# a-slide/Quade

Measured on AMD Instinct MI355X. Metric: read-pairs/sec demultiplexed (2x150 bp, dual 8 bp index), higher is better.
Workload: dtype u8

## Files before the change

quade_amd/csrc/quade_inflate3.hip:

```cpp
#include <hip/hip_runtime.h>
#include <stdint.h>
#include <stdio.h>
#include <stdlib.h>

#include "crc_lds.h"
#include "quade_inflate.h"
#include "inflate3_lane.h"
#include "quade_inflate3.h"
#include "quade_pool.h"

namespace {

using CfgS = qd3::Cfg<7, 6, 88, true, 8, 12>;
using CfgA = qd3::Cfg<8, 7, 112>;
static_assert((CfgS::LANE_DW * 64 + CfgS::RING_DW) * 4 * 4 <= 160 * 1024 - 2048, "four workgroups per CU");
static_assert((CfgA::LANE_DW * 64 + CfgA::RING_DW) * 4 * 2 <= 160 * 1024, "two workgroups per CU");

template <class C, int WPB>
__global__ __launch_bounds__(64 * WPB) void inflate3_tokens(const qd3::Unit* units, const qd_inflate3_job* jobs, uint32_t n_units, uint16_t* tokens, uint32_t* lens_scratch,
                                                            qd3::Result* res, uint32_t wait_rounds, uint32_t redo) {
    extern __shared__ __attribute__((aligned(16))) uint32_t lds_all[];
    const uint32_t lane = threadIdx.x & 63u, wave = (uint32_t)__builtin_amdgcn_readfirstlane((int)(threadIdx.x >> 6));
    uint32_t* const lds3 = lds_all + wave * (uint32_t)(C::LANE_DW * 64 + C::RING_DW);
    uint32_t* const ring = lds3;
    uint16_t* const tab = reinterpret_cast<uint16_t*>(lds3 + C::RING_DW + lane * (uint32_t)C::LANE_DW);
#pragma unroll 1
  for (uint32_t group = blockIdx.x * (uint32_t)WPB + wave; 64u * group < n_units; group += gridDim.x * (uint32_t)WPB) {
    const uint32_t u = 64u * group + lane;
    bool mine = u < n_units;
    if (redo) {
        mine = mine && res[u].status == (uint32_t)QD_INFLATE_TABLE_SPACE;
        if (!__ballot(mine)) continue;
    }
    qd3::Lane<C> L;
    {
        qd3::Unit un{nullptr, 0, ~0ull, 0, 0, 0, 0, nullptr, 0, 0};
        if (mine) {
            if (jobs) {
                const qd_inflate3_job j = jobs[u];
                const uintptr_t a = reinterpret_cast<uintptr_t>(j.payload);
                un.base = reinterpret_cast<const uint32_t*>(a & ~(uintptr_t)15);
                un.bit_start = 8ull * (a & 15u);
                un.bit_end = un.bit_start + 8ull * j.in_len;
                un.tok_off = (uint64_t)u * QD_INFLATE3_TOK_STRIDE;
                un.tok_cap = QD_INFLATE3_TOK_STRIDE;
                un.wend = (uint32_t)(((a & 15u) + j.in_len + 3u) / 4u) + 80u;
            } else {
                un = units[u];
            }
        }
        qd3::lane_init(L, un, lens_scratch + (size_t)(mine ? u : 0) * qd3::LENS_DW);
        if (!mine) {
            L.state = qd3::ST_DONE;
            L.status = 0;
        }
    }
    qd3::topup(L, ring, lane, mine);
    qd3::ring_wait();
    qd3::landed_all(L);
    qd3::prime(L, ring, lane);
    uint32_t waited = 0;
#pragma unroll 1
    for (;;) {
        const bool hdr = L.state == qd3::ST_HEADER, dec = L.state <= qd3::ST_STORED;
        const uint64_t mh = __ballot(hdr), md = __ballot(dec);
        if (!mh && !md) break;
        if (mh && (!md || waited >= wait_rounds)) {
            qd3::topup(L, ring, lane, hdr);
            qd3::ring_wait();
            qd3::landed_all(L);
            if (hdr) qd3::header<C>(L, tab, ring, lane);
            qd3::topup(L, ring, lane, L.state <= qd3::ST_STORED);
            qd3::ring_wait();
            qd3::landed_all(L);
            waited = 0;
            continue;
        }
        if (dec && qd3::bitpos(L) > L.bit_end + 64u) qd3::fail(L, QD_INFLATE_TRUNCATED);
        qd3::ring_wait();
        qd3::landed_all(L);
        qd3::topup(L, ring, lane, dec);
        if (__ballot(L.state == qd3::ST_STORED)) {
#pragma unroll 1
            for (int t = 0; t < C::ROUND_TURNS; ++t) {
                if (L.state == qd3::ST_STORED) qd3::turn_stored<C>(L, ring, lane, tokens);
                else if (L.state <= qd3::ST_DIST) qd3::turn<C>(L, tab, ring, lane, tokens);
            }
        } else {
#pragma unroll 1
            for (int t = 0; t < C::ROUND_TURNS; ++t)
                if (L.state <= qd3::ST_DIST) qd3::turn<C>(L, tab, ring, lane, tokens);
        }
        if (mh) ++waited;
    }
    if (mine) qd3::lane_finish(L, res + u);
  }
}

template <int NT, int Q>
struct R3Lds {
    uint32_t ow[16384 + 4];
    uint16_t par[Q];
    uint32_t wsum[NT / 64 + 1];
    uint32_t ctl[8];
};

template <int NT>
__device__ __forceinline__ uint32_t block_scan_excl(uint32_t v, uint32_t* wsum, uint32_t& total) {
    const uint32_t lane = threadIdx.x & 63u, wave = threadIdx.x >> 6;
    uint32_t inc = v;
#pragma unroll
    for (int d = 1; d < 64; d <<= 1) {
        const uint32_t y = __shfl_up(inc, d, 64);
        if (lane >= (uint32_t)d) inc += y;
    }
    if (lane == 63) wsum[wave] = inc;
    __syncthreads();
    uint32_t base = 0, tot = 0;
#pragma unroll
    for (int w = 0; w < NT / 64; ++w) {
        const uint32_t s = wsum[w];
        if ((uint32_t)w < wave) base += s;
        tot += s;
    }
    __syncthreads();
    total = tot;
    return base + inc - v;
}

template <int NT, int Q>
__global__ __launch_bounds__(NT) void inflate3_resolve_bgzf(const qd_inflate3_job* jobs, uint32_t n_blocks, const uint16_t* tokens, const qd3::Result* res,
                                                            int32_t* status) {
    static_assert(Q % NT == 0 && Q / NT <= 32 && 65536 % Q == 0, "a lane's share of a window");
    static_assert((size_t)Q * 2 >= 4096 + (NT / 64) * 4, "the CRC stage's tables lie where the parents were");
    constexpr int K = Q / NT;
    constexpr int CRC_SW = NT >= 1024 ? 17 : (NT >= 512 ? 33 : 65);
    static_assert((size_t)NT * CRC_SW * 4 >= 65536, "the CRC stage's slices");
    extern __shared__ __attribute__((aligned(16))) uint8_t lds_raw3[];
    R3Lds<NT, Q>& S = *reinterpret_cast<R3Lds<NT, Q>*>(lds_raw3);
    uint8_t* const ob = reinterpret_cast<uint8_t*>(S.ow);
    typedef volatile __attribute__((address_space(3))) uint8_t lds_vu8;
    typedef volatile __attribute__((address_space(3))) uint16_t lds_vu16;
    lds_vu8* const vob = (lds_vu8*)ob;
    lds_vu16* const par = (lds_vu16*)S.par;
    const uint32_t i = blockIdx.x, tid = threadIdx.x;
    if (i >= n_blocks) return;
    const qd_inflate3_job blk = jobs[i];
    const qd3::Result r = res[i];
    const uint32_t olen = blk.out_len;
    int err = (int)r.status;
    if (!err && olen > 65536u) err = QD_INFLATE_OVERRUN;
    if (!err && !r.final_seen) err = QD_INFLATE_BAD_TYPE;
    if (!err && r.text_len != olen) err = r.text_len > olen ? QD_INFLATE_OVERRUN : QD_INFLATE_LENGTH;
    if (!err && r.bit_next > 8ull * ((reinterpret_cast<uintptr_t>(blk.payload) & 15u) + (uint64_t)blk.in_len)) err = QD_INFLATE_TRUNCATED;
    if (tid < 8) S.ctl[tid] = 0;
    __syncthreads();
    if (!err) {
        const uint16_t* tk = tokens + (size_t)i * QD_INFLATE3_TOK_STRIDE;
        const uint32_t n_slots = r.n_slots;
        auto init_par = [&](uint32_t w) {
            const uint32_t qb = w * Q;
#pragma unroll
            for (int k = 0; k < K; ++k) {
                const uint32_t p = qb + tid + (uint32_t)k * NT;
                par[p - qb] = (uint16_t)p;
            }
            __syncthreads();
        };
        auto finalize = [&](uint32_t w) {
            const uint32_t qb = w * Q, hi = min(qb + (uint32_t)Q, olen);
            if (tid == 0) S.ctl[5] = S.ctl[6] = S.ctl[7] = 0;
            __syncthreads();
            uint32_t pend = 0;
#pragma unroll
            for (int k = 0; k < K; ++k) {
                const uint32_t p = qb + tid + (uint32_t)k * NT;
                if (p < hi && par[p - qb] != (uint16_t)p) pend |= 1u << k;
            }
            constexpr int MATCH_ROUNDS = 24;
#pragma unroll 1
            for (int round = 0; round < MATCH_ROUNDS; ++round) {
#pragma unroll 1
                for (uint32_t left = pend; left; left &= left - 1u) {
                    const uint32_t k = (uint32_t)__builtin_ctz(left), p = qb + tid + k * NT;
                    const uint32_t q = par[p - qb];
                    if (q < qb || par[q - qb] == q) {
                        vob[p] = vob[q];
                        par[p - qb] = (uint16_t)p;
                        pend &= ~(1u << k);
                    } else {
                        par[p - qb] = par[q - qb];
                    }
                }
                uint32_t* flag = &S.ctl[5];
                if (pend) flag[round % 3] = 1;
                __syncthreads();
                const uint32_t more = flag[round % 3];
                if (tid == 0) flag[(round + 2) % 3] = 0;
                if (!more) break;
                if (round == MATCH_ROUNDS - 1 && tid == 0) S.ctl[4] = 1;
            }
            __syncthreads();
        };
        uint32_t base_pos = 0, cur_win = 0;
        init_par(0);
#pragma unroll 1
        for (uint32_t c0 = 0; c0 < n_slots; c0 += NT * 4u) {
            const uint32_t s0 = c0 + 4u * tid;
            uint64_t four = 0;
            uint32_t prev = 0, next = 0;
            if (s0 < n_slots) {
                four = *reinterpret_cast<const uint64_t*>(tk + s0);
                if (s0) prev = tk[s0 - 1];
                if (s0 + 4u < n_slots) next = tk[s0 + 4u];
            }
            uint32_t sl[5], ln[4], at[4], sum = 0;
#pragma unroll
            for (int j = 0; j < 4; ++j) sl[j] = (uint32_t)(four >> (16 * j)) & 0xFFFFu;
            sl[4] = next;
#pragma unroll
            for (int j = 0; j < 4; ++j) {
                const bool valid = s0 + (uint32_t)j < n_slots;
                const bool is_dist = ((j ? sl[j - 1] : prev) & qd3::TOK_MATCH) != 0;
                ln[j] = (!valid || is_dist) ? 0u : ((sl[j] & qd3::TOK_MATCH) ? (sl[j] & 0xFFu) + 3u : 1u);
                sum += ln[j];
            }
            uint32_t total;
            uint32_t pos = base_pos + block_scan_excl<NT>(sum, S.wsum, total);
#pragma unroll
            for (int j = 0; j < 4; ++j) {
                at[j] = pos;
                if (ln[j] == 1u && pos < olen) ob[pos] = (uint8_t)sl[j];
                pos += ln[j];
            }
            const uint32_t chunk_hi = min(base_pos + total, olen);
            const uint32_t w_first = cur_win, w_last = max(w_first, chunk_hi ? (chunk_hi - 1u) / (uint32_t)Q : 0u);
#pragma unroll 1
            for (uint32_t w = w_first; w <= w_last; ++w) {
                if (w != cur_win) {
                    finalize(cur_win);
                    cur_win = w;
                    init_par(w);
                }
                const uint32_t wlo = w * Q, whi = min(wlo + (uint32_t)Q, olen);
#pragma unroll
                for (int j = 0; j < 4; ++j) {
                    if (ln[j] < 3u) continue;
                    const uint32_t d0 = at[j], len = ln[j], dist = sl[j + 1] + 1u;
                    if (dist > d0 || d0 + len > olen) {
                        S.ctl[4] = 1;
                        continue;
                    }
                    const uint32_t a = max(d0, wlo), z = min(d0 + len, whi);
                    for (uint32_t p = a; p < z; ++p) par[p - wlo] = (uint16_t)(p - dist);
                }
            }
            base_pos += total;
        }
        finalize(cur_win);
        if (S.ctl[4]) err = QD_INFLATE_BAD_DISTANCE;
    }
    __syncthreads();
    if (blk.check_crc) {
        uint32_t* crc_t = reinterpret_cast<uint32_t*>(S.par);
        qdcrc::stage_tables<NT>(crc_t);
        __syncthreads();
        const uint32_t crc = qdcrc::crc32_lds<NT, CRC_SW>(S.ow, err ? 0u : olen, crc_t, crc_t + 1024);
        if (!err && crc != blk.expect_crc) err = QD_INFLATE_CRC;
    }
    if (!err) {
        uint8_t* const o = blk.out;
        const uint32_t head = min(olen, (uint32_t)((4u - ((uintptr_t)o & 3u)) & 3u));
        if (tid < head) o[tid] = ob[tid];
        const uint32_t nd = (olen - head) >> 2;
        for (uint32_t k = tid; k < nd; k += NT) {
            const uint32_t a = head + 4 * k, wi = a >> 2;
            *reinterpret_cast<uint32_t*>(o + a) = __builtin_amdgcn_alignbyte(S.ow[wi + 1], S.ow[wi], a & 3u);
        }
        for (uint32_t k = head + 4 * nd + tid; k < olen; k += NT) o[k] = ob[k];
    }
    if (tid == 0) status[i] = err;
}

struct GzStretch {
    const uint32_t* base;
    uint64_t bit_from;
    uint64_t bit_to;
    uint64_t bit_end;
};

__device__ __forceinline__ uint64_t gz_bits(const uint32_t* base, uint64_t bit) {
    const uint64_t w = bit >> 5;
    const uint32_t sh = (uint32_t)bit & 31u;
    const uint64_t lo = base[w], mid = base[w + 1], hi = base[w + 2];
    return sh ? ((lo | (mid << 32)) >> sh) | (hi << (64u - sh)) : (lo | (mid << 32));
}

__device__ __forceinline__ bool gz_text_lengths_only(uint32_t a, uint32_t b) {
    b = min(b, 256u);
    if (a >= b) return true;
    const uint64_t non_text[4] = {0x00000000FFFFD9FFull, 0x8000000000000000ull, ~0ull, ~0ull};
    bool hit = false;
#pragma unroll
    for (uint32_t w = 0; w < 4; ++w) {
        const uint32_t lo = max(a, 64u * w), hi = min(b, 64u * w + 64u);
        if (lo < hi) {
            const uint64_t bits = (hi - lo == 64u ? ~0ull : ((1ull << (hi - lo)) - 1ull)) << (lo - 64u * w);
            hit = hit || (non_text[w] & bits) != 0;
        }
    }
    return !hit;
}
__device__ bool gz_header_holds(const uint32_t* base, uint64_t bit, uint64_t bit_end, uint8_t* clt, bool text_only) {
    if (bit + 17 + 12 > bit_end) return false;
    uint64_t x = gz_bits(base, bit);
    if ((x & 7u) != 4u) return false;
    const uint32_t nlit = ((uint32_t)(x >> 3) & 31u) + 257u, ndist = ((uint32_t)(x >> 8) & 31u) + 1u, ncl = ((uint32_t)(x >> 13) & 15u) + 4u;
    if (nlit > 286u || ndist > 30u) return false;
    uint64_t pos = bit + 17;
    x = gz_bits(base, pos);
    uint64_t cl = 0, cc = 0;
    for (uint32_t k = 0; k < ncl; ++k) {
        const uint32_t sym = (uint32_t)((k < 12 ? qd3::CLORDER_LO >> (5u * k) : qd3::CLORDER_HI >> (5u * (k - 12u))) & 31u);
        const uint32_t l = (uint32_t)(x >> (3u * k)) & 7u;
        cl |= (uint64_t)l << (3u * sym);
        if (l) cc += 1ull << (8u * l);
    }
    pos += 3u * ncl;
    uint64_t nx = 0;
    {
        uint32_t code = 0, kraft = 0;
#pragma unroll
        for (uint32_t l = 1; l <= 7; ++l) {
            code = (code + (l > 1 ? (uint32_t)(cc >> (8u * (l - 1u))) & 255u : 0u)) << 1;
            nx |= (uint64_t)code << (8u * l);
            kraft += ((uint32_t)(cc >> (8u * l)) & 255u) << (7u - l);
        }
        if (kraft != 128u) return false;
    }
    for (uint32_t s = 0; s < 19; ++s) {
        const uint32_t l = (uint32_t)(cl >> (3u * s)) & 7u;
        if (!l) continue;
        const uint32_t c = (uint32_t)(nx >> (8u * l)) & 255u;
        nx += 1ull << (8u * l);
        const uint32_t rev = __brev(c) >> (32u - l);
        for (uint32_t k = rev; k < 128u; k += 1u << l) clt[k] = (uint8_t)(s | (l << 5));
    }
    const uint32_t total = nlit + ndist;
    uint32_t idx = 0, prev = 0, sum_l = 0, sum_d = 0, max_l = 0, max_d = 0, n_l = 0, n_d = 0, eob = 0;
    while (idx < total) {
        if (pos + 14 > bit_end) return false;
        x = gz_bits(base, pos);
        const uint32_t e = clt[(uint32_t)x & 127u], nb = e >> 5, s = e & 31u;
        x >>= nb;
        pos += nb;
        uint32_t rep = 1, v = s;
        if (s == 16) {
            if (idx == 0) return false;
            v = prev;
            rep = 3u + ((uint32_t)x & 3u);
            pos += 2;
        } else if (s == 17) {
            v = 0;
            rep = 3u + ((uint32_t)x & 7u);
            pos += 3;
        } else if (s == 18) {
            v = 0;
            rep = 11u + ((uint32_t)x & 127u);
            pos += 7;
        }
        if (idx + rep > total) return false;
        if (v) {
            const uint32_t in_l = idx < nlit ? min(rep, nlit - idx) : 0u, in_d = rep - in_l;
            sum_l += in_l << (15u - v);
            sum_d += in_d << (15u - v);
            n_l += in_l;
            n_d += in_d;
            if (in_l) max_l = max(max_l, v);
            if (in_d) max_d = max(max_d, v);
            if (idx <= 256u && idx + rep > 256u) eob = v;
            if (sum_l > 32768u || sum_d > 32768u) return false;
            if (text_only && in_l && !gz_text_lengths_only(idx, idx + in_l)) return false;
        }
        idx += rep;
        prev = v;
    }
    if (!eob) return false;
    if (sum_l != 32768u && !(n_l == 1u && max_l == 1u)) return false;
    if (sum_d != 32768u && n_d != 0u && !(n_d == 1u && max_d == 1u)) return false;
    return true;
}

__device__ __forceinline__ bool gz_stage2(const uint32_t* base, uint64_t bit) {
    const uint32_t ncl = ((uint32_t)(gz_bits(base, bit) >> 13) & 15u) + 4u;
    const uint64_t x = gz_bits(base, bit + 17);
    uint32_t kraft = 0;
#pragma unroll
    for (uint32_t k = 0; k < 19; ++k) {
        const uint32_t l = (uint32_t)(x >> (3u * k)) & 7u;
        kraft += (k < ncl && l) ? 128u >> l : 0u;
    }
    return kraft == 128u;
}

constexpr uint32_t GZ_Q2_RUN = 16;
constexpr uint32_t GZ_Q1_CAP = 704;
constexpr uint32_t GZ_PROBE_LDS = 64 * 128 + (GZ_Q1_CAP + 128) * 4;
__global__ __launch_bounds__(64) void gz_probe(const GzStretch* stretches, uint32_t n, uint64_t* found, uint32_t text_only) {
    extern __shared__ __attribute__((aligned(16))) uint8_t probe_lds[];
    const uint32_t i = blockIdx.x, lane = threadIdx.x;
    if (i >= n) return;
    const GzStretch st = stretches[i];
    uint8_t* clt = probe_lds + 128u * lane;
    typedef volatile __attribute__((address_space(3))) uint32_t lds_vu32;
    lds_vu32* q1 = (lds_vu32*)(probe_lds + 64 * 128);
    lds_vu32* q2 = q1 + GZ_Q1_CAP;
    uint32_t n2 = 0;
    uint64_t hit = ~0ull;
    auto stage3 = [&]() {
        for (uint32_t b = 0; b < n2 && hit == ~0ull; b += 64) {
            const bool have = b + lane < n2;
            const uint64_t bit = st.bit_from + (have ? q2[b + lane] : 0u);
            const bool ok = have && gz_header_holds(st.base, bit, st.bit_end, clt, text_only != 0);
            const uint64_t m = __ballot(ok);
            if (m) hit = st.bit_from + q2[b + (uint32_t)__builtin_ctzll(m)];
        }
        n2 = 0;
    };
    const uint64_t p_end = min(st.bit_to, st.bit_end >= 29 ? st.bit_end - 28 : 0ull);
#pragma unroll 1
    for (uint64_t p0 = st.bit_from & ~31ull; p0 < p_end && hit == ~0ull; p0 += 2048) {
        const uint64_t mine = p0 + 32u * lane;
        uint32_t mask = 0;
        if (mine < p_end && mine + 32 > st.bit_from) {
            const uint64_t w = mine >> 5;
            const uint64_t two = (uint64_t)st.base[w] | ((uint64_t)st.base[w + 1] << 32);
            const uint64_t a = ~two & ~(two >> 1) & (two >> 2);
            const uint64_t hl = (two >> 4) & (two >> 5) & (two >> 6) & (two >> 7);
            const uint64_t hd = (two >> 9) & (two >> 10) & (two >> 11) & (two >> 12);
            mask = (uint32_t)(a & ~hl & ~hd);
            if (mine < st.bit_from) mask &= ~0u << (uint32_t)(st.bit_from - mine);
            if (mine + 32 > p_end) mask &= ~0u >> (uint32_t)(mine + 32 - p_end);
        }
        uint32_t cnt = (uint32_t)__popc(mask), incl = cnt;
#pragma unroll
        for (int d = 1; d < 64; d <<= 1) {
            const uint32_t y = __shfl_up(incl, d, 64);
            if (lane >= (uint32_t)d) incl += y;
        }
        const uint32_t n1 = __shfl(incl, 63, 64);
        {
            uint32_t at = incl - cnt;
            for (uint32_t m = mask; m; m &= m - 1u) q1[at++] = 32u * lane + (uint32_t)__builtin_ctz(m);
        }
        for (uint32_t b = 0; b < n1; b += 64) {
            const bool have = b + lane < n1;
            const uint64_t pos = p0 + (have ? q1[b + lane] : 0u);
            const bool ok = have && gz_stage2(st.base, pos);
            const uint64_t m = __ballot(ok);
            if (ok) q2[n2 + (uint32_t)__popcll(m & ((1ull << lane) - 1ull))] = (uint32_t)(pos - st.bit_from);
            n2 += (uint32_t)__popcll(m);
            if (n2 >= GZ_Q2_RUN) {
                stage3();
                if (hit != ~0ull) break;
            }
        }
    }
    if (hit == ~0ull) stage3();
    if (lane == 0) found[i] = hit;
}

struct GzUnit {
    uint32_t first, n;
    uint32_t stream, pad;
    uint64_t sym_off;
    uint64_t text_len;
};
constexpr uint32_t GZ_MARK = 0x8000u;
constexpr uint32_t GZ_WIN = 32768u;

template <int NT, int Q>
struct GzLds {
    uint16_t ring[GZ_WIN + Q];
    uint16_t par[Q];
    uint32_t wsum[NT / 64 + 1];
    uint32_t ctl[8];
};

template <int NT, int Q>
__global__ __launch_bounds__(NT) void gz_resolve(const GzUnit* units, uint32_t n_units, const qd3::Unit* stretches, const qd3::Result* res, const uint32_t* use_slots,
                                                 const uint16_t* tokens, uint16_t* sym, uint16_t* wout, int32_t* status) {
    static_assert(Q % NT == 0 && Q / NT <= 32 && GZ_WIN % Q == 0, "a lane's share of a window");
    constexpr int K = Q / NT;
    constexpr uint32_t RN = GZ_WIN + Q;
    extern __shared__ __attribute__((aligned(16))) uint8_t gz_lds_raw[];
    GzLds<NT, Q>& S = *reinterpret_cast<GzLds<NT, Q>*>(gz_lds_raw);
    typedef volatile __attribute__((address_space(3))) uint16_t lds_vu16;
    lds_vu16* const ring = (lds_vu16*)S.ring;
    lds_vu16* const par = (lds_vu16*)S.par;
    const uint32_t ui = blockIdx.x, tid = threadIdx.x;
    if (ui >= n_units) return;
    const GzUnit U = units[ui];
    for (uint32_t k = tid; k < GZ_WIN; k += NT) ring[k] = (uint16_t)(GZ_MARK | k);
    if (tid < 8) S.ctl[tid] = 0;
    __syncthreads();
    auto rix = [](uint32_t p) { return (p + GZ_WIN) % RN; };
    auto init_par = [&](uint32_t w) {
        const uint32_t rb = rix(w * Q);
#pragma unroll
        for (int k = 0; k < K; ++k) {
            const uint32_t i = tid + (uint32_t)k * NT;
            par[i] = (uint16_t)(rb + i);
        }
        __syncthreads();
    };
    uint16_t* const out = sym + U.sym_off;
    const uint32_t olen = (uint32_t)U.text_len;
    auto finalize = [&](uint32_t w) {
        const uint32_t qb = w * Q, hi = min(qb + (uint32_t)Q, olen), rb = rix(qb);
        if (tid == 0) S.ctl[5] = S.ctl[6] = S.ctl[7] = 0;
        __syncthreads();
        uint32_t pend = 0;
#pragma unroll
        for (int k = 0; k < K; ++k) {
            const uint32_t i = tid + (uint32_t)k * NT;
            if (qb + i < hi && par[i] != (uint16_t)(rb + i)) pend |= 1u << k;
        }
        constexpr int MATCH_ROUNDS = 24;
#pragma unroll 1
        for (int round = 0; round < MATCH_ROUNDS; ++round) {
#pragma unroll 1
            for (uint32_t left = pend; left; left &= left - 1u) {
                const uint32_t k = (uint32_t)__builtin_ctz(left), i = tid + k * NT;
                const uint32_t q = par[i];
                const bool outside = q < rb || q >= rb + (uint32_t)Q;
                if (outside || par[q - rb] == q) {
                    ring[rb + i] = ring[q];
                    par[i] = (uint16_t)(rb + i);
                    pend &= ~(1u << k);
                } else {
                    par[i] = par[q - rb];
                }
            }
            uint32_t* flag = &S.ctl[5];
            if (pend) flag[round % 3] = 1;
            __syncthreads();
            const uint32_t more = flag[round % 3];
            if (tid == 0) flag[(round + 2) % 3] = 0;
            if (!more) break;
            if (round == MATCH_ROUNDS - 1 && tid == 0) S.ctl[4] = 1;
        }
        __syncthreads();
        for (uint32_t i = tid; qb + i < hi; i += NT) out[qb + i] = ring[rb + i];
        __syncthreads();
    };
    uint32_t base_pos = 0, cur_win = 0;
    init_par(0);
#pragma unroll 1
    for (uint32_t su = U.first; su < U.first + U.n; ++su) {
        const uint16_t* tk = tokens + stretches[su].tok_off;
        const uint32_t n_slots = use_slots[su];
#pragma unroll 1
        for (uint32_t c0 = 0; c0 < n_slots; c0 += NT * 4u) {
            const uint32_t s0 = c0 + 4u * tid;
            uint64_t four = 0;
            uint32_t prev = 0, next = 0;
            if (s0 < n_slots) {
                four = *reinterpret_cast<const uint64_t*>(tk + s0);
                if (s0) prev = tk[s0 - 1];
                if (s0 + 4u < n_slots) next = tk[s0 + 4u];
            }
            uint32_t sl[5], ln[4], at[4], sum = 0;
#pragma unroll
            for (int j = 0; j < 4; ++j) sl[j] = (uint32_t)(four >> (16 * j)) & 0xFFFFu;
            sl[4] = next;
#pragma unroll
            for (int j = 0; j < 4; ++j) {
                const bool valid = s0 + (uint32_t)j < n_slots;
                const bool is_dist = ((j ? sl[j - 1] : prev) & qd3::TOK_MATCH) != 0;
                ln[j] = (!valid || is_dist) ? 0u : ((sl[j] & qd3::TOK_MATCH) ? (sl[j] & 0xFFu) + 3u : 1u);
                sum += ln[j];
            }
// ... 772 lines not shown
```

Measured before the change: 178.6 billion.

## Restructure BGZF resolve: skip match-free windows, prefetch tokens, wave-cooperative fills, wide stores

Reworks the resolve kernel's inner loop in several ways. Token chunks are prefetched one iteration ahead, with neighbour slots taken by lane shuffles. A flag carried in the block scan lets windows with no matches skip parent initialisation and pointer-jumping finalisation. Literal bytes are written with 2/4-byte stores, parent init uses 16-byte stores, and long matches are filled cooperatively by the whole wave with periodic source precomputation. Barriers become raw lgkmcnt+s_barrier and the output copy uses 16-byte global stores. Together these cut LDS traffic, barrier count and serial per-lane match fills, but they add complexity and rely on the raw barrier asm being correct.

New measurement: 179.2 billion (median of 6 runs). About the same (+0.3%).

```diff
diff --git a/quade_amd/csrc/quade_inflate3.hip b/quade_amd/csrc/quade_inflate3.hip
--- a/quade_amd/csrc/quade_inflate3.hip
+++ b/quade_amd/csrc/quade_inflate3.hip
@@ -1,4 +1,5 @@
 #include <hip/hip_runtime.h>
+#include <stddef.h>
 #include <stdint.h>
 #include <stdio.h>
 #include <stdlib.h>
@@ -128,22 +129,53 @@
     return base + inc - v;
 }
 
+__device__ __forceinline__ void r3_lds_barrier() { asm volatile("s_waitcnt lgkmcnt(0)\n\ts_barrier" ::: "memory"); }
+
+template <int NT>
+__device__ __forceinline__ uint32_t block_scan_excl_flag(uint32_t v, bool flag, uint32_t* wsum, uint32_t& total, bool& any) {
+    const uint32_t lane = threadIdx.x & 63u, wave = threadIdx.x >> 6;
+    uint32_t inc = v;
+#pragma unroll
+    for (int d = 1; d < 64; d <<= 1) {
+        const uint32_t y = __shfl_up(inc, d, 64);
+        if (lane >= (uint32_t)d) inc += y;
+    }
+    const uint32_t wave_flag = __ballot(flag) ? 0x80000000u : 0u;
+    if (lane == 63) wsum[wave] = inc | wave_flag;
+    r3_lds_barrier();
+    uint32_t base = 0, tot = 0, flags = 0;
+#pragma unroll
+    for (int w = 0; w < NT / 64; ++w) {
+        const uint32_t s = wsum[w];
+        if ((uint32_t)w < wave) base += s & 0x7FFFFFFFu;
+        tot += s & 0x7FFFFFFFu;
+        flags |= s;
+    }
+    r3_lds_barrier();
+    total = tot;
+    any = (flags & 0x80000000u) != 0;
+    return base + inc - v;
+}
+
 template <int NT, int Q>
 __global__ __launch_bounds__(NT) void inflate3_resolve_bgzf(const qd_inflate3_job* jobs, uint32_t n_blocks, const uint16_t* tokens, const qd3::Result* res,
                                                             int32_t* status) {
-    static_assert(Q % NT == 0 && Q / NT <= 32 && 65536 % Q == 0, "a lane's share of a window");
+    static_assert(Q % NT == 0 && Q / NT <= 32 && 65536 % Q == 0 && Q % 8 == 0, "a lane's share of a window");
     static_assert((size_t)Q * 2 >= 4096 + (NT / 64) * 4, "the CRC stage's tables lie where the parents were");
     constexpr int K = Q / NT;
+    constexpr int LANE_FILL = 32;
     constexpr int CRC_SW = NT >= 1024 ? 17 : (NT >= 512 ? 33 : 65);
     static_assert((size_t)NT * CRC_SW * 4 >= 65536, "the CRC stage's slices");
     extern __shared__ __attribute__((aligned(16))) uint8_t lds_raw3[];
     R3Lds<NT, Q>& S = *reinterpret_cast<R3Lds<NT, Q>*>(lds_raw3);
+    using Lds = R3Lds<NT, Q>;
+    static_assert(offsetof(Lds, par) % 16 == 0, "the parents are initialised by 16-byte stores");
     uint8_t* const ob = reinterpret_cast<uint8_t*>(S.ow);
     typedef volatile __attribute__((address_space(3))) uint8_t lds_vu8;
     typedef volatile __attribute__((address_space(3))) uint16_t lds_vu16;
     lds_vu8* const vob = (lds_vu8*)ob;
     lds_vu16* const par = (lds_vu16*)S.par;
-    const uint32_t i = blockIdx.x, tid = threadIdx.x;
+    const uint32_t i = blockIdx.x, tid = threadIdx.x, lane = tid & 63u;
     if (i >= n_blocks) return;
     const qd_inflate3_job blk = jobs[i];
     const qd3::Result r = res[i];
@@ -160,17 +192,16 @@
         const uint32_t n_slots = r.n_slots;
         auto init_par = [&](uint32_t w) {
             const uint32_t qb = w * Q;
-#pragma unroll
-            for (int k = 0; k < K; ++k) {
-                const uint32_t p = qb + tid + (uint32_t)k * NT;
-                par[p - qb] = (uint16_t)p;
-            }
-            __syncthreads();
+            uint4* const par4 = reinterpret_cast<uint4*>(S.par);
+            for (uint32_t c = tid; c < (uint32_t)Q / 8u; c += NT) {
+                const uint32_t p = qb + 8u * c, two = p | ((p + 1u) << 16);
+                par4[c] = make_uint4(two, two + 0x00020002u, two + 0x00040004u, two + 0x00060006u);
+            }
+            r3_lds_barrier();
         };
         auto finalize = [&](uint32_t w) {
             const uint32_t qb = w * Q, hi = min(qb + (uint32_t)Q, olen);
-            if (tid == 0) S.ctl[5] = S.ctl[6] = S.ctl[7] = 0;
-            __syncthreads();
+            r3_lds_barrier();
             uint32_t pend = 0;
 #pragma unroll
             for (int k = 0; k < K; ++k) {
@@ -194,55 +225,97 @@
                 }
                 uint32_t* flag = &S.ctl[5];
                 if (pend) flag[round % 3] = 1;
-                __syncthreads();
+                r3_lds_barrier();
                 const uint32_t more = flag[round % 3];
                 if (tid == 0) flag[(round + 2) % 3] = 0;
                 if (!more) break;
                 if (round == MATCH_ROUNDS - 1 && tid == 0) S.ctl[4] = 1;
             }
-            __syncthreads();
+        };
+        auto load_chunk = [&](uint32_t c0, uint64_t& four, uint32_t& edge) {
+            const uint32_t s0 = c0 + 4u * tid;
+            four = 0;
+            edge = 0;
+            if (s0 < n_slots) {
+                four = *reinterpret_cast<const uint64_t*>(tk + s0);
+                const uint32_t at_edge = lane == 0 ? s0 - 1u : s0 + 4u;
+                if (lane == 0 ? s0 != 0 : (lane == 63 && at_edge < n_slots)) edge = tk[at_edge];
+            }
         };
         uint32_t base_pos = 0, cur_win = 0;
-        init_par(0);
+        bool dirty = false;
+        uint64_t four_ahead;
+        uint32_t edge_ahead;
+        load_chunk(0, four_ahead, edge_ahead);
 #pragma unroll 1
         for (uint32_t c0 = 0; c0 < n_slots; c0 += NT * 4u) {
             const uint32_t s0 = c0 + 4u * tid;
-            uint64_t four = 0;
-            uint32_t prev = 0, next = 0;
-            if (s0 < n_slots) {
-                four = *reinterpret_cast<const uint64_t*>(tk + s0);
-                if (s0) prev = tk[s0 - 1];
-                if (s0 + 4u < n_slots) next = tk[s0 + 4u];
-            }
+            const uint64_t four = four_ahead;
+            const uint32_t edge = edge_ahead;
+            if (c0 + NT * 4u < n_slots) load_chunk(c0 + NT * 4u, four_ahead, edge_ahead);
             uint32_t sl[5], ln[4], at[4], sum = 0;
 #pragma unroll
             for (int j = 0; j < 4; ++j) sl[j] = (uint32_t)(four >> (16 * j)) & 0xFFFFu;
+            uint32_t prev = __shfl_up(sl[3], 1, 64), next = __shfl_down(sl[0], 1, 64);
+            if (lane == 0) prev = edge;
+            if (lane == 63) next = edge;
             sl[4] = next;
+            bool has_match = false;
 #pragma unroll
             for (int j = 0; j < 4; ++j) {
                 const bool valid = s0 + (uint32_t)j < n_slots;
                 const bool is_dist = ((j ? sl[j - 1] : prev) & qd3::TOK_MATCH) != 0;
                 ln[j] = (!valid || is_dist) ? 0u : ((sl[j] & qd3::TOK_MATCH) ? (sl[j] & 0xFFu) + 3u : 1u);
+                has_match = has_match || ln[j] >= 3u;
                 sum += ln[j];
             }
             uint32_t total;
-            uint32_t pos = base_pos + block_scan_excl<NT>(sum, S.wsum, total);
+            bool chunk_match;
+            uint32_t pos = base_pos + block_scan_excl_flag<NT>(sum, has_match, S.wsum, total, chunk_match);
 #pragma unroll
             for (int j = 0; j < 4; ++j) {
                 at[j] = pos;
-                if (ln[j] == 1u && pos < olen) ob[pos] = (uint8_t)sl[j];
                 pos += ln[j];
+            }
+            {
+                const bool l0 = ln[0] == 1u, l1 = ln[1] == 1u, l2 = ln[2] == 1u, l3 = ln[3] == 1u;
+                const uint32_t b01 = (sl[0] & 0xFFu) | ((sl[1] & 0xFFu) << 8), b23 = (sl[2] & 0xFFu) | ((sl[3] & 0xFFu) << 8);
+                if (l0 && l1 && l2 && l3 && at[0] + 4u <= olen) {
+                    const uint32_t v = b01 | (b23 << 16);
+                    __builtin_memcpy(ob + at[0], &v, 4);
+                } else {
+                    if (l0 && l1 && at[0] + 2u <= olen) {
+                        const uint16_t v = (uint16_t)b01;
+                        __builtin_memcpy(ob + at[0], &v, 2);
+                    } else {
+                        if (l0 && at[0] < olen) ob[at[0]] = (uint8_t)sl[0];
+                        if (l1 && at[1] < olen) ob[at[1]] = (uint8_t)sl[1];
+                    }
+                    if (l2 && l3 && at[2] + 2u <= olen) {
+                        const uint16_t v = (uint16_t)b23;
+                        __builtin_memcpy(ob + at[2], &v, 2);
+                    } else {
+                        if (l2 && at[2] < olen) ob[at[2]] = (uint8_t)sl[2];
+                        if (l3 && at[3] < olen) ob[at[3]] = (uint8_t)sl[3];
+                    }
+                }
             }
             const uint32_t chunk_hi = min(base_pos + total, olen);
             const uint32_t w_first = cur_win, w_last = max(w_first, chunk_hi ? (chunk_hi - 1u) / (uint32_t)Q : 0u);
 #pragma unroll 1
             for (uint32_t w = w_first; w <= w_last; ++w) {
                 if (w != cur_win) {
-                    finalize(cur_win);
+                    if (dirty) finalize(cur_win);
                     cur_win = w;
+                    dirty = false;
+                }
+                if (!chunk_match) continue;
+                if (!dirty) {
                     init_par(w);
+                    dirty = true;
                 }
                 const uint32_t wlo = w * Q, whi = min(wlo + (uint32_t)Q, olen);
+                uint32_t by_wave = 0;
 #pragma unroll
                 for (int j = 0; j < 4; ++j) {
                     if (ln[j] < 3u) continue;
@@ -252,15 +325,42 @@
                         continue;
                     }
                     const uint32_t a = max(d0, wlo), z = min(d0 + len, whi);
-                    for (uint32_t p = a; p < z; ++p) par[p - wlo] = (uint16_t)(p - dist);
+                    if (a >= z) continue;
+                    if (z - a > (uint32_t)LANE_FILL) by_wave |= 1u << j;
+                    const uint32_t z_mine = min(z, a + (uint32_t)LANE_FILL);
+                    uint32_t off = a - d0;
+                    if (off >= dist) off %= dist;
+                    uint32_t src = d0 - dist + off;
+                    for (uint32_t p = a; p < z_mine; ++p) {
+                        par[p - wlo] = (uint16_t)src;
+                        if (++src == d0) src = d0 - dist;
+                    }
                 }
+#pragma unroll
+                for (int j = 0; j < 4; ++j) {
+                    uint64_t m = __ballot((by_wave >> j) & 1u);
+                    while (m) {
+                        const int from = __builtin_ctzll(m);
+                        m &= m - 1ull;
+                        const uint32_t d0 = (uint32_t)__builtin_amdgcn_readlane((int)at[j], from), len = (uint32_t)__builtin_amdgcn_readlane((int)ln[j], from);
+                        const uint32_t dist = (uint32_t)__builtin_amdgcn_readlane((int)sl[j + 1], from) + 1u;
+                        const uint32_t a = max(d0, wlo) + (uint32_t)LANE_FILL, z = min(d0 + len, whi), first = d0 - dist;
+                        if (dist >= len) {
+                            for (uint32_t p = a + lane; p < z; p += 64u) par[p - wlo] = (uint16_t)(p - dist);
+                        } else if (dist == 1u) {
+                            for (uint32_t p = a + lane; p < z; p += 64u) par[p - wlo] = (uint16_t)first;
+                        } else {
+                            for (uint32_t p = a + lane; p < z; p += 64u) par[p - wlo] = (uint16_t)(first + (p - d0) % dist);
+                        }
+                    }
+                }
             }
             base_pos += total;
         }
-        finalize(cur_win);
-        if (S.ctl[4]) err = QD_INFLATE_BAD_DISTANCE;
+        if (dirty) finalize(cur_win);
     }
     __syncthreads();
+    if (!err && S.ctl[4]) err = QD_INFLATE_BAD_DISTANCE;
     if (blk.check_crc) {
         uint32_t* crc_t = reinterpret_cast<uint32_t*>(S.par);
         qdcrc::stage_tables<NT>(crc_t);
@@ -270,14 +370,16 @@
     }
     if (!err) {
         uint8_t* const o = blk.out;
-        const uint32_t head = min(olen, (uint32_t)((4u - ((uintptr_t)o & 3u)) & 3u));
+        const uint32_t head = min(olen, (uint32_t)((16u - ((uintptr_t)o & 15u)) & 15u));
         if (tid < head) o[tid] = ob[tid];
-        const uint32_t nd = (olen - head) >> 2;
-        for (uint32_t k = tid; k < nd; k += NT) {
-            const uint32_t a = head + 4 * k, wi = a >> 2;
-            *reinterpret_cast<uint32_t*>(o + a) = __builtin_amdgcn_alignbyte(S.ow[wi + 1], S.ow[wi], a & 3u);
-        }
-        for (uint32_t k = head + 4 * nd + tid; k < olen; k += NT) o[k] = ob[k];
+        const uint32_t n16 = (olen - head) >> 4, sh = head & 3u;
+        for (uint32_t k = tid; k < n16; k += NT) {
+            const uint32_t a = head + 16u * k, wi = a >> 2;
+            const uint32_t w0 = S.ow[wi], w1 = S.ow[wi + 1], w2 = S.ow[wi + 2], w3 = S.ow[wi + 3], w4 = S.ow[wi + 4];
+            *reinterpret_cast<uint4*>(o + a) = make_uint4(__builtin_amdgcn_alignbyte(w1, w0, sh), __builtin_amdgcn_alignbyte(w2, w1, sh),
+                                                          __builtin_amdgcn_alignbyte(w3, w2, sh), __builtin_amdgcn_alignbyte(w4, w3, sh));
+        }
+        for (uint32_t k = head + 16u * n16 + tid; k < olen; k += NT) o[k] = ob[k];
     }
     if (tid == 0) status[i] = err;
 }
```
